# sqlp/sedumi

Hardware: AMD Instinct MI355X
Metric: IPM iters/sec (ADA' form+factor+solve) (higher is better)
Workload: dtype f64; 1 GPU; control07.mat: examples/control07.mat (BASELINE.json configs[1]), m=666, nnz(At)=107940, nnz(ADA')=443556, nnz(L)=222111; unit = getada1+2+3, blkchol, 4x(fwblkslv,./d,bwblkslv); parallelism=single GPU

## Files before the change

### sedumi_amd/csrc/sdm_ada.hip

```cpp
#include "sdm_plan.h"
#include <algorithm>
#include <cmath>
#include <cstdlib>

namespace sdm {

__global__ void k_dsqr(double *dsqr, const int *code, const double *dl, const double *ddet, int nlq) {
  int r = blockIdx.x * blockDim.x + threadIdx.x;
  if (r < nlq) { int c = code[r]; dsqr[r] = c == -1 ? dl[r] : (c >= 0 ? ddet[c] : -ddet[-2 - c]); }
}
__global__ void k_fill(double *x, double v, int64_t n) {
  int64_t t = (int64_t)blockIdx.x * blockDim.x + threadIdx.x;
  int64_t stride = (int64_t)gridDim.x * blockDim.x;
  for (; t < n; t += stride) x[t] = v;
}

constexpr int SPDOT_CAP = 2048;
template <int LPE>
__global__ void __launch_bounds__(256)
k_ada_spdot(double *ada, const int64_t *ADAjc, const int *ADAir, const int64_t *Mbeg, const int64_t *Mend,
            const int *Mir, const double *Mpr, const double *wgt, const int *invperm, int accumulate, int jbase, int cap) {
  SDM_DYN_SMEM(smem);
  double *jv = (double *)smem;
  int *jr = (int *)(jv + cap);
// ... 238 lines not shown
            if (part) { ar -= x * di; ai += x * dr; } else { ar += x * dr; ai += x * di; }
          }
        }
        Y[t * n + i] = ar;
        Dl[t * n + i] = D[(int64_t)col * n + i];
        if (herm) { Yi[t * n + i] = ai; Dli[t * n + i] = -Di[(int64_t)col * n + i]; }
      }
    }
    __syncthreads();
    if (!herm) {
      double sreg[S1_TREG];
#pragma unroll
      for (int k = 0; k < S1_TREG; k++) sreg[k] = 0.0;
#pragma unroll 1
      for (int t = 0; t < cc; t++) {
        const double *Yt = Y + t * n, *Dt = Dl + t * n;
#pragma unroll
        for (int k = 0; k < S1_TREG; k++) sreg[k] += Yt[rreg[k]] * Dt[creg[k]] + Yt[creg[k]] * Dt[rreg[k]];
      }
#pragma unroll
      for (int k = 0; k < S1_TREG; k++) zreg[k] += sreg[k] / 2;
    }
    for (int u = nreg + tid; u < ulen; u += bs) {
      int q = U[u];
      const int zpart = q >= n * n ? 1 : 0;
      q -= zpart * n * n;
      const int c = q / n, r = q - c * n;
      double v;
      if (!herm) {
        double a1 = 0.0, a2 = 0.0;
        for (int t = 0; t < cc; t++) {
          a1 += Y[t * n + r] * Dl[t * n + c];
          a2 += Y[t * n + c] * Dl[t * n + r];
        }
        v = (a1 + a2) / 2;
      } else {
        double rrc = 0.0, irc = 0.0, rcr = 0.0, icr = 0.0;
        for (int t = 0; t < cc; t++) {
          const double drc = Dl[t * n + c], dic = Dli[t * n + c], drr = Dl[t * n + r], dir = Dli[t * n + r];
          const double yr_r = Y[t * n + r], yi_r = Yi[t * n + r], yr_c = Y[t * n + c], yi_c = Yi[t * n + c];
          rrc += yr_r * drc - yi_r * dic; irc += yr_r * dic + yi_r * drc;
          rcr += yr_c * drr - yi_c * dir; icr += yr_c * dir + yi_c * drr;
        }
        v = zpart ? (irc - icr) / 2 : (rrc + rcr) / 2;
      }
      if (c0 == 0) z[u] = v; else z[u] += v;
    }
    __syncthreads();
  }
  if (!herm && R2.ada && ulen <= S1_TREG * bs) {
    double *zl = Y;
#pragma unroll
    for (int k = 0; k < S1_TREG; k++) if (tid + k * bs < ulen) zl[tid + k * bs] = zreg[k];
    __syncthreads();
    const int j = R2.t_col[task], kblk = T.t_blk[task];
    const int ipj = R2.invperm ? R2.invperm[j] : 0;
    for (int64_t e = R2.ADAjc[j] + tid; e < R2.ADAjc[j + 1]; e += bs) {
      const int i = R2.ADAir[e];
      if (R2.invperm && R2.invperm[i] > ipj) continue;
      double acc = 0.0, aabs = 0.0;
      int64_t p = R2.Ajc_psd[i];
      const int64_t pe = R2.Ajc[i + 1];
      for (; p + 4 <= pe; p += 4) {
        double x[4]; int b[4], u[4];
#pragma unroll
        for (int q = 0; q < 4; q++) { x[q] = R2.Apr[p + q]; b[q] = R2.Ablk[p + q]; u[q] = R2.Aupos[p + q]; }
#pragma unroll
        for (int q = 0; q < 4; q++) if (b[q] == kblk) { const double term = x[q] * zl[u[q]]; acc += term; aabs += fabs(term); }
      }
      for (; p < pe; p++) if (R2.Ablk[p] == kblk) { const double term = R2.Apr[p] * zl[R2.Aupos[p]]; acc += term; aabs += fabs(term); }
      const double base = R2.ada[e];
      R2.ada[e] = base + acc;
      if (i == j) R2.absd[j] = base + aabs;
    }
    return;
  }
  if (!herm) {
#pragma unroll
    for (int k = 0; k < S1_TREG; k++) if (tid + k * bs < ulen) z[tid + k * bs] = zreg[k];
  }
}

__global__ void __launch_bounds__(64 * S1_WAVES, 3 * S1_WAVES / 4)
k_psd_stage1_mfma(Stage1Tab T, const double *udsqr, double *zbuf, int ldsY, int nzcap, int task0, const int *order, double *zero_ptr, long long zero_n) {
  SDM_DYN_SMEM(smem);
  for (long long i = (long long)blockIdx.x * blockDim.x + threadIdx.x; i < zero_n; i += (long long)gridDim.x * blockDim.x) zero_ptr[i] = 0.0;
  const int task = order ? order[blockIdx.x] : blockIdx.x + task0;
  const int n = T.t_n[task], nslot = T.t_nslot[task], ulen = T.t_ulen[task];
  const int np = (n + 15) & ~15, nt = np >> 4, ntile = nt * nt;
  double *Yl = (double *)smem;
  double *Dl = Yl + S1_KC * np;
  double *Zl = (double *)smem;
  const int ldz = n | 1;
  const int64_t slot0 = T.t_slotptr[task], tend = T.t_end[task];
  const double *D = udsqr + T.t_udoff[task];
  double *z = zbuf + T.t_zoff[task];
  const int64_t rowbase = T.psd_start[T.t_blk[task]];
  const int tid = threadIdx.x, bs = blockDim.x;
  const int wave = SDM_UNIFORM_INT(tid >> 6), lane = tid & 63, nw = bs >> 6;
  const int li = lane & 15, lk = lane >> 4;
  const int rcpn = ((1 << 20) + n - 1) / n;
  static_assert(S1_KC * S1_MAXN * S1_MAXN < (1 << 20) && S1_KC % 4 == 0, "k_psd_stage1_mfma: reciprocal division, four slots per MFMA step");
  sdm_double4 acc[S1_MAXT];
  for (int x = 0; x < S1_MAXT; x++) for (int r = 0; r < 4; r++) acc[x][r] = 0.0;
  double *nzx = (double *)smem + ldsY;
  int *nzr = (int *)(nzx + nzcap);
  __shared__ int sbeg[S1_MAXN + 1], scol[S1_MAXN];
  SDM_PHASE_BEGIN();
  const int64_t nzb = T.s_nzptr[slot0];
  const bool staged = tend - nzb <= nzcap && nslot <= S1_MAXN;
  if (staged) {
    for (int64_t u = nzb + tid; u < tend; u += bs) { nzx[u - nzb] = T.Apr[u]; nzr[u - nzb] = (int)(T.Air[u] - rowbase); }
    for (int t = tid; t <= nslot; t += bs) sbeg[t] = (int)((t < nslot ? T.s_nzptr[slot0 + t] : tend) - nzb);
    for (int t = tid; t < nslot; t += bs) scol[t] = T.s_col[slot0 + t];
  }
  __syncthreads();
  SDM_PHASE(0);
  for (int t = wave; t < S1_KC; t += nw)
    if (lane < np - n) { Yl[t * np + n + lane] = 0.0; Dl[t * np + n + lane] = 0.0; }
  for (int c0 = 0; c0 < nslot; c0 += S1_KC) {
    const int cc = min(S1_KC, nslot - c0), kq = (cc + 3) & ~3;
    for (int e = tid; e < cc * n; e += bs) {
      const int t = (e * rcpn) >> 20, i = e - t * n;
      int sb, se, col;
      if (staged) { sb = sbeg[c0 + t]; se = sbeg[c0 + t + 1]; col = scol[c0 + t]; }
      else {
        sb = (int)(T.s_nzptr[slot0 + c0 + t] - nzb);
        se = (int)(((c0 + t + 1 < nslot) ? T.s_nzptr[slot0 + c0 + t + 1] : tend) - nzb);
        col = T.s_col[slot0 + c0 + t];
      }
      double a = 0.0;
      if (staged) {
        int u = sb;
        for (; u + 4 <= se; u += 4) {
          const double d0 = D[(int64_t)(nzr[u] - col * n) * n + i], d1 = D[(int64_t)(nzr[u + 1] - col * n) * n + i];
          const double d2 = D[(int64_t)(nzr[u + 2] - col * n) * n + i], d3 = D[(int64_t)(nzr[u + 3] - col * n) * n + i];
          a += nzx[u] * d0; a += nzx[u + 1] * d1; a += nzx[u + 2] * d2; a += nzx[u + 3] * d3;
        }
        for (; u < se; u++) a += nzx[u] * D[(int64_t)(nzr[u] - col * n) * n + i];
      } else {
        for (int64_t u = nzb + sb; u < nzb + se; u++) a += T.Apr[u] * D[(int64_t)((int)(T.Air[u] - rowbase) - col * n) * n + i];
      }
      Yl[t * np + i] = a;
      Dl[t * np + i] = D[(int64_t)col * n + i];
    }
    for (int t = cc + wave; t < kq; t += nw)
      for (int i = lane; i < n; i += 64) { Yl[t * np + i] = 0.0; Dl[t * np + i] = 0.0; }
    SDM_PHASE(1);
    __syncthreads();
    SDM_PHASE(2);
    for (int x = 0; x < S1_MAXT; x++) {
      const int tile = wave + x * nw;
      if (tile < ntile) {
        const int I = tile / nt, J = tile - I * nt;
        int npo = np; SDM_PIN(npo);
        const double *Ya = Yl + lk * npo + I * 16 + li, *Db = Dl + lk * npo + J * 16 + li;
        int q = 0;
        for (; q + 4 <= kq / 4; q += 4) {
          double a[4], b[4];
#pragma unroll
          for (int k = 0; k < 4; k++) { a[k] = Ya[4 * (q + k) * npo]; b[k] = Db[4 * (q + k) * npo]; }
#pragma unroll
          for (int k = 0; k < 4; k++) acc[x] = SDM_MFMA_F64_16x16x4(a[k], b[k], acc[x]);
        }
        for (; q < kq / 4; q++) acc[x] = SDM_MFMA_F64_16x16x4(Ya[4 * q * npo], Db[4 * q * npo], acc[x]);
      }
    }
    SDM_PHASE(3);
    __syncthreads();
    SDM_PHASE(4);
  }
  for (int x = 0; x < S1_MAXT; x++) {
    const int tile = wave + x * nw;
    if (tile < ntile) {
      const int I = tile / nt, J = tile - I * nt;
      for (int r = 0; r < 4; r++)
        if (I * 16 + lk + 4 * r < n && J * 16 + li < n) Zl[(I * 16 + lk + 4 * r) * ldz + J * 16 + li] = acc[x][r];
    }
  }
  __syncthreads();
  SDM_PHASE(5);
  const int *RC = T.u_rc + T.t_uoff[task];
  for (int u0 = 0; u0 < ulen; u0 += 8 * bs) {
    int rc[8];
#pragma unroll
    for (int x = 0; x < 8; x++) rc[x] = RC[min(u0 + x * bs + tid, ulen - 1)];
#pragma unroll
    for (int x = 0; x < 8; x++) {
      const int u = u0 + x * bs + tid;
      const int r = rc[x] >> 16, c = rc[x] & 0xffff;
      if (u < ulen) z[u] = (Zl[r * ldz + c] + Zl[c * ldz + r]) / 2;
    }
  }
  SDM_PHASE(6);
#if defined(SDM_PHASES) && !defined(SDM_EMU)
  if (tid == 0) { atomicAdd(&sdm_phase_acc[30], 1ull); if (n > 40) atomicAdd(&sdm_phase_acc[31], 1ull); }
#endif
}

__global__ void __launch_bounds__(256)
k_psd_stage2(double *ada, double *absd, const int64_t *ADAjc, const int *ADAir, const int64_t *Ajc,
             const int64_t *Ajc_psd, const double *Apr, const int *Ablk, const int *Aupos,
             const int64_t *c_taskptr, const int *t_blk, const int64_t *t_zoff, const int64_t *c_zlen, const double *zbuf,
             const int *invperm, int nblk, int thread_per_row, int jbase, int zlds) {
  SDM_DYN_SMEM(smem);
  long long *zo = (long long *)smem;
  double *zl = (double *)(zo + nblk);
  const int j = blockIdx.x + jbase;
  const int tid = threadIdx.x, bs = blockDim.x;
  const int64_t tb0 = c_taskptr[j], te0 = c_taskptr[j + 1];
  const bool jhas = te0 > tb0;
  const int64_t z0 = jhas ? t_zoff[tb0] : 0;
  const int64_t zlen = c_zlen[j];
  for (int k = tid; k < nblk; k += bs) zo[k] = -1;
  __syncthreads();
  for (int64_t t = tb0 + tid; t < te0; t += bs) zo[t_blk[t]] = t_zoff[t] - z0;
  const bool staged = thread_per_row && jhas && zlen <= zlds;
  if (staged)
    for (int64_t u = tid; u < zlen; u += bs) zl[u] = zbuf[z0 + u];
  __syncthreads();
  const double *zsrc = staged ? zl : zbuf + z0;
  const int ipj = invperm ? invperm[j] : 0;
  if (thread_per_row) {
    for (int64_t e = ADAjc[j] + tid; e < ADAjc[j + 1]; e += bs) {
      const int i = ADAir[e];
      if (invperm && invperm[i] > ipj) continue;
      double acc = 0.0, aabs = 0.0;
      if (jhas) {
        int64_t t = Ajc_psd[i];
        const int64_t te = Ajc[i + 1];
        for (; t + 4 <= te; t += 4) {
          double x[4]; int b[4], u[4];
#pragma unroll
          for (int q = 0; q < 4; q++) { x[q] = Apr[t + q]; b[q] = Ablk[t + q]; u[q] = Aupos[t + q]; }
#pragma unroll
          for (int q = 0; q < 4; q++) {
            const long long off = zo[b[q]];
            if (off >= 0) { const double term = x[q] * zsrc[off + u[q]]; acc += term; aabs += fabs(term); }
          }
        }
        for (; t < te; t++) {
          const long long off = zo[Ablk[t]];
          if (off >= 0) { const double term = Apr[t] * zsrc[off + Aupos[t]]; acc += term; aabs += fabs(term); }
        }
      }
      const double base = ada[e];
      ada[e] = base + acc;
      if (i == j) absd[j] = jhas ? base + aabs : 0.0;
    }
  } else {
    const int wave = tid >> 6, lane = tid & 63, nw = bs >> 6;
    for (int64_t e = ADAjc[j] + wave; e < ADAjc[j + 1]; e += nw) {
      const int i = ADAir[e];
      if (invperm && invperm[i] > ipj) continue;
      double acc = 0.0, aabs = 0.0;
      if (jhas)
        for (int64_t t = Ajc_psd[i] + lane; t < Ajc[i + 1]; t += 64) {
          const long long off = zo[Ablk[t]];
          if (off >= 0) { const double term = Apr[t] * zsrc[off + Aupos[t]]; acc += term; aabs += fabs(term); }
        }
      for (int off = 32; off > 0; off >>= 1) { acc += __shfl_down(acc, off); aabs += __shfl_down(aabs, off); }
      if (lane == 0) {
        const double base = ada[e];
        ada[e] = base + acc;
        if (i == j) absd[j] = jhas ? base + aabs : 0.0;
// ... 423 lines not shown
}
static Stage1Tab stage1_tab(const AdaPlan &A) {
  Stage1Tab T;
  T.t_n = A.t_n.p; T.t_nslot = A.t_nslot.p; T.t_ulen = A.t_ulen.p; T.t_herm = A.t_herm.p; T.s_col = A.s_col.p;
  T.u_pos = A.u_pos.p; T.u_rc = A.u_rc.p; T.Air = A.d_Air.p; T.t_slotptr = A.t_slotptr.p; T.t_udoff = A.t_udoff.p; T.t_uoff = A.t_uoff.p;
  T.t_zoff = A.t_zoff.p; T.t_end = A.t_end.p; T.s_nzptr = A.s_nzptr.p; T.Apr = A.d_Apr.p; T.t_blk = A.t_blk.p;
  T.psd_start = A.d_psd_start.p;
  return T;
}
static Stage2Ride stage2_ride(sdm_plan *P, double *ada, const int *d_invperm) {
  const AdaPlan &A = P->ada;
  Stage2Ride R2 = {};
  R2.ada = ada; R2.absd = P->absd.p; R2.ADAjc = A.d_ADAjc.p; R2.Ajc = A.d_Ajc.p; R2.Ajc_psd = A.d_Ajc_psd.p; R2.ADAir = A.d_ADAir.p;
  R2.Ablk = A.d_Ablk.p; R2.Aupos = A.d_Aupos.p; R2.t_col = A.t_col.p; R2.invperm = d_invperm; R2.Apr = A.d_Apr.p;
  return R2;
}
template <int JB>
static void launch_stage2_ell(sdm_plan *P, double *ada, const int *d_invperm, int ncols, int jbase, bool sym, int gsplit, bool cleared) {
  AdaPlan &A = P->ada;
  const size_t lds = (size_t)JB * (size_t)A.zmax * sizeof(double);
#ifndef SDM_EMU
  if (lds > 48 * 1024) SDM_HIP_CHECK(hipFuncSetAttribute((const void *)k_psd_stage2_ell<JB>, hipFuncAttributeMaxDynamicSharedMemorySize, (int)lds));
#endif
  SDM_KLAUNCH_AS(P, P->stream, JB == 4 ? "k_psd_stage2_ell<4>" : JB == 2 ? "k_psd_stage2_ell<2>" : "k_psd_stage2_ell<1>", k_psd_stage2_ell<JB>,
                 dim3((ncols + JB - 1) / JB, gsplit), dim3(64 * ELL_WAVES), lds, ada, P->absd.p, A.d_ADAjc.p, A.d_ADAir.p,
                 A.d_Ajc.p, A.d_Ajc_psd.p, A.d_Apr.p, A.d_Ablk.p, A.d_Aupos.p, A.c_taskptr.p, A.t_blk.p, A.t_ulen.p,
                 A.t_zoff.p, A.zbuf.p, A.d_uoff.p, A.g_row.p, A.g_len.p, A.g_off.p, A.g_val.p, A.g_bu.p, A.ell_ng, d_invperm,
                 (int)A.zmax, (int)A.m, jbase, jbase + ncols, A.ell_pos.p, sym ? (const int *)A.ell_order.p : (const int *)nullptr,
                 A.d_Azpos.p, A.t_zdst.p, cleared ? 1 : 0,
                 sym ? (const long long *)A.cdp64.p : (const long long *)A.cdc64.p, sym ? (const int *)A.cdp32.p : (const int *)A.cdc32.p);
}
void ada_psd(sdm_plan *P, double *ada, const int *d_invperm, bool sym_input, bool absd_done) {
  AdaPlan &A = P->ada;
  const int m = (int)A.m;
  if (A.sdpN == 0 || sym_input || A.col1 <= A.col0) ada_zero_flush(P);
  if (A.sdpN == 0) {
    if (sym_input) symmetrize_in_place(P, ada);
    if (!absd_done) SDM_KLAUNCH(P, k_diag, dim3((m + 255) / 256), dim3(256), 0, P->absd.p, ada, A.d_ADAjc.p, A.d_ADAir.p, m);
    return;
  }
  if (A.col1 <= A.col0) return;
  const int ncols = (int)(A.col1 - A.col0), jbase = (int)A.col0;
  const int task0 = (int)A.h_taskptr[A.col0], ntask = (int)(A.h_taskptr[A.col1] - A.h_taskptr[A.col0]);
  const size_t direct_lds = (size_t)(2 * A.sdpN + 2 * S1_DIRECT_MAXNZ * A.sdpN + 2) * sizeof(int) + (size_t)(2 * A.sdpN) * sizeof(long long) +
                            (size_t)(S1_DIRECT_MAXNZ * A.sdpN) * sizeof(double);
  const bool direct = A.thread_per_row && !A.ell_ok && A.sdpN == A.rsdpN && A.s1_maxnz <= S1_DIRECT_MAXNZ && direct_lds <= S1_DIRECT_LDS_MAX;
  const bool direct_zero = direct && !sym_input && !d_invperm && A.zero_ptr == ada + P->ada_jc[A.col0] &&
                           A.zero_n == (long long)(P->ada_jc[A.col1] - P->ada_jc[A.col0]);
  if (direct_zero) { A.zero_ptr = nullptr; A.zero_n = 0; }
  const bool s1_mfma = A.maxn <= S1_MAXN && A.sdpN == A.rsdpN;
  if (direct || ntask <= 0 || !s1_mfma) ada_zero_flush(P);
  if (direct) {
    if (sym_input) symmetrize_in_place(P, ada);
    const int nb = (int)A.sdpN;
    const size_t lds_cols = (size_t)DIRECT_JB * (direct_lds + 16) + (size_t)A.sdpN * sizeof(int);
    if (!d_invperm && (int64_t)(P->ada_jc[A.col1] - P->ada_jc[A.col0]) == (int64_t)ncols * m && lds_cols <= S1_DIRECT_LDS_MAX) {
      const int ysplit = std::max(1, std::min(16, (int)((m + 511) / 512)));
      SDM_KLAUNCH(P, k_psd_direct_cols, dim3((ncols + DIRECT_JB - 1) / DIRECT_JB, ysplit), dim3(256), lds_cols, ada, P->absd.p, A.d_ADAjc.p, A.d_Ajc.p, A.d_Ajc_psd.p, A.d_Apr.p,
                  A.d_Air.p, A.d_Ablk.p, A.c_taskptr.p, A.t_blk.p, A.t_n.p, A.t_udoff.p, A.t_slotptr.p, A.s_nzptr.p, A.t_end.p, A.d_psd_start.p, A.udsqr.p,
                  nb, jbase, jbase + ncols, m, direct_zero ? 1 : 0);
    } else
      SDM_KLAUNCH(P, k_psd_direct, dim3(ncols), dim3(256), direct_lds, ada, P->absd.p, A.d_ADAjc.p, A.d_ADAir.p, A.d_Ajc.p, A.d_Ajc_psd.p, A.d_Apr.p, A.d_Air.p,
                  A.d_Ablk.p, A.c_taskptr.p, A.t_blk.p, A.t_n.p, A.t_udoff.p, A.t_slotptr.p, A.s_nzptr.p, A.t_end.p, A.d_psd_start.p, A.udsqr.p,
                  d_invperm, nb, jbase, direct_zero ? 1 : 0);
    SDM_HIP_CHECK(hipGetLastError());
    return;
  }
  bool stage1_cleared_all = false;
  if (ntask > 0) {
    const Stage1Tab T = stage1_tab(A);
#ifndef SDM_EMU
    SDM_HIP_CHECK(hipFuncSetAttribute((const void *)k_psd_stage1, hipFuncAttributeMaxDynamicSharedMemorySize, (int)A.stage1_lds));
#endif
    const int nzcap = s1_nzcap(A.s1_maxnz);
    if (s1_mfma) {
      const int ldsy = s1_mfma_ldsy(A.maxn);
      const size_t lds = s1_mfma_lds(A.maxn, A.s1_maxnz);
#ifndef SDM_EMU
      if (lds > 48 * 1024) SDM_HIP_CHECK(hipFuncSetAttribute((const void *)k_psd_stage1_mfma, hipFuncAttributeMaxDynamicSharedMemorySize, (int)lds));
#endif
      double *zp = A.zero_ptr; const long long zn = A.zero_n;
      A.zero_ptr = nullptr; A.zero_n = 0;
      stage1_cleared_all = zp == ada + P->ada_jc[A.col0] && zn == (long long)(P->ada_jc[A.col1] - P->ada_jc[A.col0]);
      SDM_KLAUNCH(P, k_psd_stage1_mfma, dim3((unsigned)ntask), dim3(64 * S1_WAVES), lds, T, A.udsqr.p, A.zbuf.p, ldsy, nzcap, task0,
                  (ntask == (int)A.ntask) ? (const int *)A.t_order.p : (const int *)nullptr, zp, zn);
    } else {
      const size_t one = (size_t)(A.sdpN > A.rsdpN ? 4 : 2) * (size_t)A.maxn * sizeof(double);
      const size_t ldsy = std::max(one, std::min(A.stage1_lds, (size_t)S1_GEN_LDS));
      const size_t lds = ldsy + (size_t)nzcap * (sizeof(double) + sizeof(int));
#ifndef SDM_EMU
      SDM_HIP_CHECK(hipFuncSetAttribute((const void *)k_psd_stage1, hipFuncAttributeMaxDynamicSharedMemorySize, (int)lds));
#endif
      const bool ride = A.one_task_per_col && A.thread_per_row && !A.ell_ok && A.sdpN == A.rsdpN && A.s1_maxulen <= 6 * 512 &&
                        (int64_t)A.s1_maxulen * (int64_t)sizeof(double) <= (int64_t)ldsy;
      if (ride) {
        if (sym_input) symmetrize_in_place(P, ada);
        SDM_HIP_CHECK(hipMemsetAsync(P->absd.p + jbase, 0, (size_t)ncols * sizeof(double), P->stream));
      }
      SDM_KLAUNCH(P, k_psd_stage1, dim3((unsigned)ntask), dim3(512), lds, T, A.udsqr.p, A.zbuf.p, (int)(ldsy / sizeof(double)), task0, nzcap,
                  ride ? stage2_ride(P, ada, d_invperm) : Stage2Ride{},
                  (ntask == (int)A.ntask && A.t_order_xcd.n == (size_t)ntask) ? (const int *)A.t_order_xcd.p : (const int *)nullptr);
      if (ride) { SDM_HIP_CHECK(hipGetLastError()); return; }
    }
  }
  if (sym_input) symmetrize_in_place(P, ada);
  if (A.ell_ok) {
    const bool sym = A.ell_full && !d_invperm && jbase == 0 && ncols == m;
    const int gsplit = sym ? 3 : 1;
    const bool cleared = stage1_cleared_all && !sym_input;
    const size_t zbytes = (size_t)A.zmax * sizeof(double);
    if (4 * zbytes <= 64 * 1024 && m >= 1024) launch_stage2_ell<4>(P, ada, d_invperm, ncols, jbase, sym, gsplit, cleared);
    else if (2 * zbytes <= 64 * 1024 && m >= 512) launch_stage2_ell<2>(P, ada, d_invperm, ncols, jbase, sym, gsplit, cleared);
    else launch_stage2_ell<1>(P, ada, d_invperm, ncols, jbase, sym, gsplit, cleared);
  } else {
    const int64_t zl = (A.thread_per_row && A.zmaxj * 8 <= 64 * 1024) ? A.zmaxj : 0;
    const size_t lds = (size_t)A.sdpN * 8 + (size_t)zl * 8;
#ifndef SDM_EMU
    if (lds > 48 * 1024) SDM_HIP_CHECK(hipFuncSetAttribute((const void *)k_psd_stage2, hipFuncAttributeMaxDynamicSharedMemorySize, (int)lds));
#endif
    SDM_KLAUNCH(P, k_psd_stage2, dim3(ncols), dim3(256), lds, ada, P->absd.p, A.d_ADAjc.p, A.d_ADAir.p, A.d_Ajc.p,
               A.d_Ajc_psd.p, A.d_Apr.p, A.d_Ablk.p, A.d_Aupos.p, A.c_taskptr.p, A.t_blk.p, A.t_zoff.p, A.c_zlen.p, A.zbuf.p,
               d_invperm, (int)A.sdpN, A.thread_per_row ? 1 : 0, jbase, (int)zl);
  }
  SDM_HIP_CHECK(hipGetLastError());
}

}

#if defined(SDM_PHASES) && !defined(SDM_EMU)
extern "C" int sdm_debug_phases_ada(unsigned long long *out32, int reset) {
  if (out32 && hipMemcpyFromSymbol(out32, HIP_SYMBOL(sdm_phase_acc), 32 * sizeof(unsigned long long)) != hipSuccess) return 1;
  if (reset) { unsigned long long z[32] = {0}; if (hipMemcpyToSymbol(HIP_SYMBOL(sdm_phase_acc), z, sizeof(z)) != hipSuccess) return 1; }
  return 0;
}
#endif
```

### sedumi_amd/csrc/sdm_ada_build.hip

```cpp
#include "sdm_plan.h"
#include <algorithm>

namespace sdm {
namespace {

struct AdaIn {
  sdm_int m; const sdm_int *Ajc, *Air; const double *Apr; const sdm_int *Ajc_psd;
  sdm_int lpN, lorN, sdpN, rsdpN; const sdm_int *sdpNL, *qblkstart, *psd_blkstart, *Qjc, *Qir, *ADAjc, *ADAir;
  sdm_int psd_begin(sdm_int j) const { return sdpN > 0 ? Ajc_psd[j] : Ajc[j + 1]; }
};
struct PsdPatterns {
  std::vector<int> Ablk, Aupos;
  std::vector<std::vector<int>> U;
  std::vector<int64_t> uoff;
  sdm_int psdnnz = 0;
};
struct Stage1Tasks {
  std::vector<int> t_col, t_blk, t_n, t_nslot, t_ulen, t_herm, s_col, order, order_xcd;
  std::vector<int64_t> t_slotptr, t_udoff, t_uoff, t_zoff, t_end, s_nzptr, c_taskptr, c_zlen;
};

void upload_narrow(DevBuf<int> &d, const sdm_int *h, sdm_int n) { std::vector<int> v((size_t)n); for (sdm_int t = 0; t < n; t++) v[t] = (int)h[t]; d.upload(v); }

PsdPatterns psd_patterns(AdaPlan &A, const AdaIn &in) {
// ... 152 lines not shown
    }
  A.ell_ng = ng;
  A.g_row.upload(grow); A.g_len.upload(glen); A.g_off.upload(goff); A.g_val.upload(gval); A.g_bu.upload(gbu);
  { std::vector<int> pos((size_t)m); for (sdm_int p = 0; p < m; p++) pos[(size_t)order[p]] = (int)p; A.ell_pos.upload(pos); }
  A.ell_order.upload(order);
  A.ell_full = (in.ADAjc[m] == (sdm_int)m * m);
  A.d_uoff.upload(pt.uoff); A.d_Azpos.upload(zp); A.t_zdst.upload(zd);
  ell_column_records(in, tk, zd, nullptr, A.cdc64, A.cdc32);
  ell_column_records(in, tk, zd, order.data(), A.cdp64, A.cdp32);
  A.ell_ok = true;
}

std::vector<int> ada_transpose_map(const AdaIn &in) {
  const sdm_int m = in.m, *ADAjc = in.ADAjc, *ADAir = in.ADAir;
  std::vector<int> adaT((size_t)ADAjc[m], -1);
  for (sdm_int j = 0; j < m; j++)
    for (sdm_int e = ADAjc[j]; e < ADAjc[j + 1]; e++) {
      sdm_int i = ADAir[e];
      const sdm_int *b = ADAir + ADAjc[i], *en = ADAir + ADAjc[i + 1];
      const sdm_int *f = std::lower_bound(b, en, j);
      if (f != en && *f == j) adaT[e] = (int)(f - ADAir);
    }
  return adaT;
}

void lq_dense_forms(AdaPlan &A, const AdaIn &in) {
  const sdm_int m = in.m, lorN = in.lorN;
  sdm_int nz = 0;
  for (sdm_int j = 0; j < m; j++) nz += in.Ajc_psd[j] - in.Ajc[j];
  const double cells = (double)A.nlq * (double)m;
  A.lq_dense = A.nlq > 0 && m > 1 && nz > 0 && (double)nz >= 0.10 * cells && cells * 8.0 <= 1.0e9;
  A.q_dense = lorN > 0 && A.nnzQ > 0 && (double)A.nnzQ >= 0.10 * (double)lorN * (double)m && (double)lorN * m * 8.0 <= 1.0e9;
  if (A.lq_dense) {
    std::vector<double> D((size_t)A.nlq * (size_t)m, 0.0);
    for (sdm_int j = 0; j < m; j++)
      for (sdm_int t = in.Ajc[j]; t < in.Ajc_psd[j]; t++) D[(size_t)j * (size_t)A.nlq + (size_t)in.Air[t]] = in.Apr[t];
    A.Alq_d.upload(D);
  } else A.Alq_d.release();
  if (A.q_dense) {
    std::vector<int64_t> dst((size_t)A.nnzQ);
    for (sdm_int j = 0; j < m; j++)
      for (sdm_int t = in.Qjc[j]; t < in.Qjc[j + 1]; t++) dst[(size_t)t] = (int64_t)j * lorN + in.Qir[t];
    A.q_dst.upload(dst);
    A.Q_d.alloc((size_t)lorN * (size_t)m);
    if (A.lq_dense && (double)lorN * (double)m <= 1.6e7) {
      std::vector<int> src((size_t)lorN * (size_t)m, -1);
      for (sdm_int t = 0; t < A.nnzQ; t++) src[(size_t)dst[(size_t)t]] = (int)t;
      A.q_src.upload(src);
    } else A.q_src.release();
  } else { A.Q_d.release(); A.q_dst.release(); A.q_src.release(); }
  if (A.lq_dense || A.q_dense) {
    const int nt = (int)((m + TILE - 1) / TILE), T = nt * (nt + 1) / 2;
    const sdm_int rows = std::max(A.lq_dense ? A.nlq : 0, A.q_dense ? lorN : 0);
    A.gram_split = (int)std::max<sdm_int>(1, std::min<sdm_int>((rows + TILE - 1) / TILE, std::max(1, 512 / T)));
    A.gram_part.alloc((size_t)A.gram_split * (size_t)m * (size_t)m);
  } else A.gram_part.release();
}

void upload_tables(AdaPlan &A, const AdaIn &in, const PsdPatterns &pt, const Stage1Tasks &tk, const std::vector<int> &adaT) {
  const sdm_int m = in.m, lorN = in.lorN, sdpN = in.sdpN;
  { std::vector<int> code((size_t)A.nlq, -1);
    for (sdm_int r = in.lpN; r < in.lpN + lorN && r < A.nlq; r++) code[r] = (int)(-2 - (r - in.lpN));
    for (sdm_int k = 0; k < lorN; k++)
      for (sdm_int r = in.qblkstart[k]; r < in.qblkstart[k + 1] && r < A.nlq; r++) code[r] = (int)k;
    A.dsqr_code.upload(code); }
  A.d_Ajc.upload(in.Ajc, (size_t)m + 1); A.d_Ajc_psd.upload(in.Ajc_psd, (size_t)m);
  upload_narrow(A.d_Air, in.Air, A.nnzA);
  A.d_Apr.upload(in.Apr, (size_t)A.nnzA);
  A.d_Ablk.upload(pt.Ablk); A.d_Aupos.upload(pt.Aupos);
  { std::vector<int64_t> v(m + 1, 0); if (lorN > 0) v.assign(in.Qjc, in.Qjc + m + 1); A.d_Qjc.upload(v); }
  upload_narrow(A.d_Qir, in.Qir, A.nnzQ);
  A.d_ADAjc.upload(in.ADAjc, (size_t)m + 1);
  upload_narrow(A.d_ADAir, in.ADAir, in.ADAjc[m]);
  A.d_ADAT.upload(adaT);
  { std::vector<int> upos((size_t)pt.uoff[sdpN]), urc(upos.size(), 0);
    for (sdm_int k = 0; k < sdpN; k++) std::copy(pt.U[k].begin(), pt.U[k].end(), upos.begin() + pt.uoff[k]);
    for (sdm_int k = 0; k < std::min(sdpN, in.rsdpN); k++) {
      const int n = (int)A.psd_n[k];
      if (n >= 65536) continue;
      for (size_t u = 0; u < pt.U[k].size(); u++) { const int q = pt.U[k][u], c = q / n, r = q - c * n; urc[(size_t)pt.uoff[k] + u] = (r << 16) | c; }
    }
    A.u_pos.upload(upos); A.u_rc.upload(urc); }
  A.t_col.upload(tk.t_col); A.t_blk.upload(tk.t_blk); A.t_n.upload(tk.t_n); A.t_nslot.upload(tk.t_nslot); A.t_ulen.upload(tk.t_ulen);
  A.t_herm.upload(tk.t_herm); A.t_order.upload(tk.order);
  if (tk.order_xcd.empty()) A.t_order_xcd.release(); else A.t_order_xcd.upload(tk.order_xcd);
  A.t_slotptr.upload(tk.t_slotptr); A.t_udoff.upload(tk.t_udoff); A.t_uoff.upload(tk.t_uoff); A.t_zoff.upload(tk.t_zoff);
  A.s_col.upload(tk.s_col); A.s_nzptr.upload(tk.s_nzptr); A.c_taskptr.upload(tk.c_taskptr); A.c_zlen.upload(tk.c_zlen);
  A.t_end.upload(tk.t_end);
  { std::vector<int64_t> v(A.psd_start.begin(), A.psd_start.end()); if (v.empty()) v.push_back(0); A.d_psd_start.upload(v); }
  { std::vector<int64_t> v(lorN + 1, A.nlq); for (sdm_int k = 0; k <= lorN && lorN > 0; k++) v[k] = in.qblkstart[k]; A.d_qblk.upload(v); }
  A.zbuf.alloc((size_t)std::max<int64_t>(A.zlen, 1));
  A.dsqr.alloc((size_t)std::max<sdm_int>(A.nlq, 1));
  A.dl.alloc((size_t)std::max<sdm_int>(in.lpN, 1)); A.ddet.alloc((size_t)std::max<sdm_int>(lorN, 1));
  A.qpr.alloc((size_t)std::max<sdm_int>(A.nnzQ, 1)); A.udsqr.alloc((size_t)std::max<sdm_int>(A.lenud, 1));
  A.q1.alloc((size_t)std::max<sdm_int>(lorN, 1));
  A.q2.alloc((size_t)std::max<sdm_int>(lorN > 0 ? in.qblkstart[lorN] - in.qblkstart[0] : 0, 1));
  A.symtmp.alloc((size_t)std::max<sdm_int>(in.ADAjc[m], 1));
  const size_t need = (size_t)(sdpN > in.rsdpN ? 4 : 2) * (size_t)A.maxn * sizeof(double);
  A.stage1_lds = std::max<size_t>(96 * 1024, need);
  if (A.stage1_lds > 136 * 1024) throw std::runtime_error("PSD block too large for the LDS-staged D*A*D kernel (n > 8700)");
}

}

void ada_build(sdm_plan *P, sdm_int N, sdm_int m, const sdm_int *Ajc, const sdm_int *Air, const double *Apr, const sdm_int *Ajc_psd, sdm_int lpN,
               sdm_int lorN, sdm_int sdpN, sdm_int rsdpN, const sdm_int *sdpNL, const sdm_int *qblkstart, const sdm_int *psd_blkstart,
               const sdm_int *Qjc, const sdm_int *Qir, const sdm_int *ADAjc, const sdm_int *ADAir) {
  AdaPlan &A = P->ada;
  const AdaIn in = {m, Ajc, Air, Apr, Ajc_psd, lpN, lorN, sdpN, rsdpN, sdpNL, qblkstart, psd_blkstart, Qjc, Qir, ADAjc, ADAir};
  A.N = N; A.m = m; A.nnzA = Ajc[m]; A.lpN = lpN; A.lorN = lorN; A.sdpN = sdpN; A.rsdpN = rsdpN;
  A.ic_n.release(); A.ufac.release();
  if (A.nnzA >= (sdm_int)1 << 31 || N >= (sdm_int)1 << 31) throw std::runtime_error("At too large for 32-bit row indices");
  A.nlq = sdpN > 0 ? psd_blkstart[0] : N;
  if (lorN > 0 && qblkstart[lorN] != A.nlq && sdpN > 0) throw std::runtime_error("qblkstart / psd_blkstart mismatch");
  const PsdPatterns pt = psd_patterns(A, in);
  A.thread_per_row = (m > 0 && pt.psdnnz / (double)m < 48.0);
  A.nnz_lq = A.nnzA - pt.psdnnz;
  A.nnzQ = lorN > 0 ? Qjc[m] : 0;
  A.lq_maxcol = 0; A.q_maxcol = 0;
  for (sdm_int j = 0; j < m; j++) A.lq_maxcol = std::max<int64_t>(A.lq_maxcol, in.psd_begin(j) - Ajc[j]);
  for (sdm_int j = 0; j < m && lorN > 0; j++) A.q_maxcol = std::max<int64_t>(A.q_maxcol, Qjc[j + 1] - Qjc[j]);
  const Stage1Tasks tk = stage1_tasks(A, in, pt);
  stage2_ell(A, in, pt, tk);
  upload_tables(A, in, pt, tk, ada_transpose_map(in));
  lq_dense_forms(A, in);
  P->has_ada = true;
}

}
```

### sedumi_amd/csrc/sdm_plan.h

```cpp
#pragma once
#include "../../include/sedumi_hip.h"
#include "sdm_rt.h"
#include <mutex>
#include <string>
#include <vector>

namespace sdm {

constexpr int NB = 64;
constexpr int TILE = 64;
constexpr int UTP = 72;
constexpr int S1_MAXN = 96;
constexpr int S1_KC = 32;
constexpr int S1_WAVES = 8;
constexpr int S1_NZ = 1536;
constexpr int s1_nzcap(int64_t maxnz) { return (int)(((maxnz + 1) & ~(int64_t)1) < S1_NZ ? ((maxnz + 1) & ~(int64_t)1) : S1_NZ); }
constexpr int s1_mfma_ldsy(int maxn) { return 2 * S1_KC * ((maxn + 15) & ~15) > maxn * (maxn | 1) ? 2 * S1_KC * ((maxn + 15) & ~15) : maxn * (maxn | 1); }
constexpr size_t s1_mfma_lds(int maxn, int64_t maxnz) { return (size_t)s1_mfma_ldsy(maxn) * sizeof(double) + (size_t)s1_nzcap(maxnz) * (sizeof(double) + sizeof(int)); }
constexpr int S1_MAXT = ((S1_MAXN / 16) * (S1_MAXN / 16) + S1_WAVES - 1) / S1_WAVES;
constexpr int S1_GEN_LDS = 74 * 1024;
constexpr int ELL_WAVES = 8;
constexpr int SOLVE_LDS_MAX = 3072;
constexpr int FUSE_MAX_TILES = 1 << 20;
constexpr int SBW_MIN = 256;
constexpr int SBW_MAX = 2048;
constexpr int SINV_MAXLEV = 4;
constexpr int SPREP_NCNT = 2 + 2 * SINV_MAXLEV;
constexpr int SROWS = 16;
#ifndef SDM_SW
#define SDM_SW 8
#endif
constexpr int SW = SDM_SW;
constexpr int LDL_THREADS = 512;
constexpr int PANEL_THREADS = 256;
constexpr int ROWS_BATCH = 16 * (PANEL_THREADS / 64);
constexpr int TRSM_ROWS = 128;
#ifndef SDM_MFMA_MIN_ROWS
#define SDM_MFMA_MIN_ROWS 48
#endif
constexpr int MFMA_MIN_ROWS = SDM_MFMA_MIN_ROWS;
constexpr int CHK = 16;
constexpr int64_t ASM_FULL_MAX = 4 << 20;
constexpr int FRONT_MAXT = 64;
constexpr int FRONT_XCNT_OFF = 2 * FRONT_MAXT + FRONT_MAXT * FRONT_MAXT;
constexpr int FRONT_CNT = FRONT_XCNT_OFF + FRONT_MAXT * FRONT_MAXT;
constexpr int FRONT_POOL = 1;
constexpr int PANEL_RB = (LDL_THREADS / 64) * NB * 17;
constexpr size_t PANEL_LDS = (size_t)(NB * (NB + 1) + PANEL_RB) * sizeof(double);
constexpr size_t PANEL_LDS_RIDE = std::max(PANEL_LDS, (size_t)4 * NB * UTP * sizeof(double));
constexpr int FRONT_CV_OFF = NB * (NB + 1) + (LDL_THREADS / 64) * NB * 17;
constexpr size_t FRONT_LDS = (size_t)(FRONT_CV_OFF + NB * TILE) * sizeof(double);
static_assert(PANEL_RB >= NB * NB && PANEL_RB >= (NB - CHK) * TRSM_ROWS && TRSM_ROWS == 16 * (LDL_THREADS / 64) && ROWS_BATCH <= TRSM_ROWS, "panel LDS layout");

template <class T>
struct DevBuf {
  T *p = nullptr;
  size_t n = 0;
  DevBuf() = default;
  DevBuf(const DevBuf &) = delete;
  DevBuf &operator=(const DevBuf &) = delete;
  DevBuf(DevBuf &&o) noexcept : p(o.p), n(o.n) { o.p = nullptr; o.n = 0; }
  DevBuf &operator=(DevBuf &&o) noexcept { if (this != &o) { release(); p = o.p; n = o.n; o.p = nullptr; o.n = 0; } return *this; }
  ~DevBuf() { release(); }
  void release() {
    if (p) (void)hipFree(p);
    p = nullptr; n = 0;
  }
  void alloc(size_t count) {
    release();
    n = count;
    SDM_HIP_CHECK(hipMalloc((void **)&p, (count ? count : 1) * sizeof(T)));
  }
  void upload(const std::vector<T> &h) {
    alloc(h.size());
    if (!h.empty()) SDM_HIP_CHECK(hipMemcpy(p, h.data(), h.size() * sizeof(T), hipMemcpyHostToDevice));
  }
  void upload(const T *h, size_t count) {
    alloc(count);
    if (count) SDM_HIP_CHECK(hipMemcpy(p, h, count * sizeof(T), hipMemcpyHostToDevice));
  }
};

struct PanelCtx {
  double *lb; const double *ubp; int *pivstat; double *pivval; double *colbuf; const double *ada; const int *asm_src; const int64_t *Ljc;
  int mtot, pad;
};

struct HostFlag {
  int *host = nullptr;
  HostFlag() = default;
  HostFlag(const HostFlag &) = delete;
  HostFlag &operator=(const HostFlag &) = delete;
  HostFlag(HostFlag &&o) noexcept : host(o.host) { o.host = nullptr; }
  HostFlag &operator=(HostFlag &&o) noexcept { if (this != &o) { if (host) (void)hipHostFree(host); host = o.host; o.host = nullptr; } return *this; }
  ~HostFlag() { if (host) (void)hipHostFree(host); }
  void ensure() {
    if (host) return;
    SDM_HIP_CHECK(hipHostMalloc((void **)&host, 4 * sizeof(int), 0));
    for (int i = 0; i < 4; i++) host[i] = 0;
  }
  int *dev() {
    ensure();
// ... 46 lines not shown
  std::vector<int> childptr, childlist, levptr, levlist, lev_T;
  std::vector<char> sn_active;
  double pars_canceltol = 0, pars_maxu = 0, pars_abstol = 0; int pars_use_absd = 0;
  bool begun = false;
  std::vector<LevelLaunch> launches;
  std::vector<int> lev_first_launch;
  DevBuf<int> d_first, d_ns, d_ms, d_ld, d_parent, d_childptr, d_childlist, d_levlist, d_lindx, d_relidx, d_perm;
  DevBuf<int64_t> d_foff, d_xl, d_woff, d_roff, d_toff, d_asm_dst, d_asm_dstT, d_Ljc;
  DevBuf<int> d_asm_src;
  DevBuf<double> fronts, frontsT, wvec, colbuf, d, dsolve, lb, pivval, ub;
  DevBuf<int> pivstat;
  DevBuf<int> diag_cnt;
  DevBuf<int> d_asm_fsrc;
  DevBuf<int> front_cnt;
  DevBuf<int> d_fslot;
  std::vector<char> lev_persist;
  std::vector<int> lev_maxT;
  std::vector<int> lev_ntw;
  DevBuf<int> upd_cnt;
  DevBuf<double> panelrec;
  DevBuf<PanelCtx> panel_ctx;
  PanelCtx panel_ctx_host = {};
  HostFlag tmo;
  int *sweep_tmo() { return tmo.dev() + 1; }
  int sbw = SBW_MIN;
  int sbw_req = 0;
  bool front_off_req = false;
  bool sprep_off = false;
  int tile_wgs_req = 0;
  int64_t ssize = 0; int nsbtot = 0;
  std::vector<int64_t> sn_soff; std::vector<int> sn_sld, sn_sboff;
  DevBuf<int64_t> d_soff; DevBuf<int> d_sld, d_sboff;
  DevBuf<double> S, xfin, zdiv;
  DevBuf<double> ST;
  DevBuf<double> LT;
  std::vector<int64_t> sn_ltoff; DevBuf<int64_t> d_ltoff;
  DevBuf<int> l_lt; int n_lt = 0;
  DevBuf<double> Tarena;
  DevBuf<int> sweep_cnt;
  DevBuf<unsigned long long> sb_g;
  DevBuf<int> l_i128, l_items;
  int n_i128 = 0, n_items = 0;
  bool follow = false;
  bool front_disabled = false;
  bool merge_disabled = false;
  std::vector<int> lev_followT;
  std::vector<int> stage_ptr;
  std::vector<SolveLevel> slev;
  DevBuf<double> prep_part; DevBuf<int> prep_ticket;
  double growth_max = 1e4;
  double growth_used = 1e4;
  double refine_max = 1e10;
  int refine_mode = 1;
  bool refine_on = false;
  int sweep_seq = 0;
  HostFlag noted;
};

struct FrontTab {
  const int *first, *ns, *ms, *ld;
  const int64_t *foff, *xl, *woff, *roff, *toff;
  const int *childptr, *childlist, *lindx, *relidx;
  const int64_t *soff; const int *sld, *sboff;
  const int64_t *ltoff = nullptr;
  const int *fslot = nullptr;
  int one = 0, o_s = 0, o_ns = 0, o_ms = 0, o_ld = 0, o_first = 0, o_sld = 0, o_sboff = 0;
  int64_t o_foff = 0, o_soff = 0, o_woff = 0, o_xl = 0, o_ltoff = 0;
};

struct AdaPlan {
  sdm_int N = 0, m = 0, nnzA = 0, lpN = 0, lorN = 0, sdpN = 0, rsdpN = 0;
  sdm_int nlq = 0;
  sdm_int lenud = 0, ntask = 0, zlen = 0, nnzQ = 0, nnz_lq = 0;
  int maxn = 0;
  bool thread_per_row = false;
  sdm_int col0 = 0, col1 = 0;
  double *zero_ptr = nullptr; long long zero_n = 0; bool zero_defer = false;
  std::vector<int64_t> h_taskptr;
  std::vector<sdm_int> psd_n, psd_start, psd_udoff;
  DevBuf<int64_t> d_Ajc, d_Ajc_psd, d_Qjc, d_ADAjc;
  DevBuf<int> d_Air, d_Qir, d_ADAir, d_ADAT;
  DevBuf<double> d_Apr;
  DevBuf<int> d_Ablk, d_Aupos;
  DevBuf<int> t_col, t_blk, t_n, t_nslot, t_ulen, t_herm, t_order, t_order_xcd;
  DevBuf<int64_t> t_slotptr, t_udoff, t_uoff, t_zoff;
  DevBuf<int> s_col;
  DevBuf<int64_t> s_nzptr;
  int64_t s1_maxnz = 0;
  int64_t lq_maxcol = 0, q_maxcol = 0;
  bool one_task_per_col = false;
  int s1_maxulen = 0;
  DevBuf<int> u_rc;
  DevBuf<int> u_pos;
  DevBuf<int64_t> c_taskptr;
  DevBuf<double> zbuf, dsqr, symtmp;
  DevBuf<int> dsqr_code;
  bool lq_dense = false, q_dense = false;
  int gram_split = 1;
  DevBuf<double> Alq_d, Q_d, gram_part;
  DevBuf<int64_t> q_dst;
  DevBuf<int> q_src;
  DevBuf<int64_t> t_end, d_psd_start;
  DevBuf<double> dl, ddet, qpr, udsqr;
  DevBuf<double> q1, q2;
  DevBuf<int64_t> d_qblk;
  DevBuf<double> ufac;
  DevBuf<int> ic_n, ic_poff, ic_perm; DevBuf<int64_t> ic_off;
  PinnedInts ic_perm_host; bool ic_has_perm = false;
  std::vector<sdm_int> h_Ajc, h_Air; std::vector<double> h_Apr;
  bool pcg_ready = false;
  DevBuf<int64_t> d_Tjc, pb_off; DevBuf<int> d_Tir, pb_n, pb_herm, pb_poff, pb_items, aden_cols;
  DevBuf<double> d_Tpr, xN, psd, psdtmp, aden;
  int pcg_ntiles = 0, aden_n = 0;
  DevBuf<double> wp_rv, wp_rb, qauxdet, qauxtr, wp_y, wp_dx, wp_r, wp_work, wp_part, wp_sc;
  PinnedInts wp_host;
  size_t stage1_lds = 0;
  bool ell_ok = false;
  int ell_ng = 0;
  int64_t zmax = 0, zmaxj = 0;
  DevBuf<int64_t> c_zlen;
  DevBuf<int> g_row, g_len, g_bu;
  DevBuf<long long> cdc64, cdp64;
  DevBuf<int> cdc32, cdp32;
  DevBuf<int> d_Azpos, t_zdst;
  DevBuf<int> ell_pos;
  DevBuf<int> ell_order;
  bool ell_full = false;
  DevBuf<int64_t> g_off, d_uoff;
  DevBuf<double> g_val;
};

}

namespace sdm {
struct KProf {
  bool enabled = false;
  struct Rec { const char *name; hipEvent_t a, b; };
  std::vector<Rec> recs;
  std::vector<hipEvent_t> pool;
  hipEvent_t get() {
    if (!pool.empty()) { hipEvent_t e = pool.back(); pool.pop_back(); return e; }
    hipEvent_t e; SDM_HIP_CHECK(hipEventCreate(&e)); return e;
  }
};
}

namespace sdm {
struct DensePlan {
  sdm_int nden = 0, dznnz = 0, pnnz = 0, mrows = 0;
  bool active = false, factored = false;
  bool tables_on_host = false;
  std::vector<sdm_int> LADjc, LADir, dzjc, dzir, colperm, first;
  std::vector<int64_t> poff, betajc, permoff;
  std::vector<int> dopiv;
  std::vector<int> later_ptr;
  DevBuf<int> d_dzir, d_colperm, d_pivperm, d_dopiv, d_later;
  DevBuf<int64_t> d_dzjc, d_poff, d_betajc, d_permoff;
  DevBuf<double> ad, lad, wvb, p, beta, dgat, smult, dden;
  DevBuf<double> w_psq, w_mu, w_key;
  DevBuf<int> w_ord, w_ord2, w_acc, w_post, w_dep, w_st;
};
}

struct sdm_plan {
  int device = 0;
  sdm::DensePlan dense;
  sdm::KProf kprof;
// ... 171 lines not shown
```

Before: 2828 IPM iters/s.

## Pack stage-1 task metadata into 64-byte records and prefetch D gathers

Per-task metadata for the PSD stage-1 MFMA kernel now lives in one 64-byte record, with an array pre-permuted into the launch order. Each block does a single contiguous load instead of a chain of dependent gathers through order, t_* and psd_start. The staged gather loop is software-pipelined so the next element's first D value and diagonal are fetched while the current one accumulates. It also moves index arithmetic to 32-bit unsigned offsets, which assumes the offsets fit in 32 bits.

```diff
diff --git a/sedumi_amd/csrc/sdm_ada.hip b/sedumi_amd/csrc/sdm_ada.hip
--- a/sedumi_amd/csrc/sdm_ada.hip
+++ b/sedumi_amd/csrc/sdm_ada.hip
@@ -344,23 +344,21 @@
 }
 
 __global__ void __launch_bounds__(64 * S1_WAVES, 3 * S1_WAVES / 4)
-k_psd_stage1_mfma(Stage1Tab T, const double *udsqr, double *zbuf, int ldsY, int nzcap, int task0, const int *order, double *zero_ptr, long long zero_n) {
+k_psd_stage1_mfma(Stage1Tab T, const S1Rec *recs, const double *udsqr, double *zbuf, int ldsY, int nzcap, int rec0, double *zero_ptr, long long zero_n) {
   SDM_DYN_SMEM(smem);
   for (long long i = (long long)blockIdx.x * blockDim.x + threadIdx.x; i < zero_n; i += (long long)gridDim.x * blockDim.x) zero_ptr[i] = 0.0;
-  const int task = order ? order[blockIdx.x] : blockIdx.x + task0;
-  const int n = T.t_n[task], nslot = T.t_nslot[task], ulen = T.t_ulen[task];
+  const S1Rec rec = recs[blockIdx.x + rec0];
+  const int n = rec.n, nslot = rec.nslot, ulen = rec.ulen;
   const int np = (n + 15) & ~15, nt = np >> 4, ntile = nt * nt;
   double *Yl = (double *)smem;
   double *Dl = Yl + S1_KC * np;
   double *Zl = (double *)smem;
   const int ldz = n | 1;
-  const int64_t slot0 = T.t_slotptr[task], tend = T.t_end[task];
-  const double *D = udsqr + T.t_udoff[task];
-  double *z = zbuf + T.t_zoff[task];
-  const int64_t rowbase = T.psd_start[T.t_blk[task]];
+  const int slot0 = rec.slot0, tend = rec.tend, rowbase = rec.rowbase;
+  const double *D = udsqr + rec.udoff;
+  double *z = zbuf + rec.zoff;
   const int tid = threadIdx.x, bs = blockDim.x;
   const int wave = SDM_UNIFORM_INT(tid >> 6), lane = tid & 63, nw = bs >> 6;
-  const int li = lane & 15, lk = lane >> 4;
   const int rcpn = ((1 << 20) + n - 1) / n;
   static_assert(S1_KC * S1_MAXN * S1_MAXN < (1 << 20) && S1_KC % 4 == 0, "k_psd_stage1_mfma: reciprocal division, four slots per MFMA step");
   sdm_double4 acc[S1_MAXT];
@@ -369,10 +367,10 @@
   int *nzr = (int *)(nzx + nzcap);
   __shared__ int sbeg[S1_MAXN + 1], scol[S1_MAXN];
   SDM_PHASE_BEGIN();
-  const int64_t nzb = T.s_nzptr[slot0];
+  const int nzb = rec.nzb;
   const bool staged = tend - nzb <= nzcap && nslot <= S1_MAXN;
   if (staged) {
-    for (int64_t u = nzb + tid; u < tend; u += bs) { nzx[u - nzb] = T.Apr[u]; nzr[u - nzb] = (int)(T.Air[u] - rowbase); }
+    for (int u = nzb + tid; u < tend; u += bs) { nzx[u - nzb] = T.Apr[u]; nzr[u - nzb] = T.Air[u] - rowbase; }
     for (int t = tid; t <= nslot; t += bs) sbeg[t] = (int)((t < nslot ? T.s_nzptr[slot0 + t] : tend) - nzb);
     for (int t = tid; t < nslot; t += bs) scol[t] = T.s_col[slot0 + t];
   }
@@ -382,32 +380,55 @@
     if (lane < np - n) { Yl[t * np + n + lane] = 0.0; Dl[t * np + n + lane] = 0.0; }
   for (int c0 = 0; c0 < nslot; c0 += S1_KC) {
     const int cc = min(S1_KC, nslot - c0), kq = (cc + 3) & ~3;
-    for (int e = tid; e < cc * n; e += bs) {
-      const int t = (e * rcpn) >> 20, i = e - t * n;
-      int sb, se, col;
-      if (staged) { sb = sbeg[c0 + t]; se = sbeg[c0 + t + 1]; col = scol[c0 + t]; }
-      else {
-        sb = (int)(T.s_nzptr[slot0 + c0 + t] - nzb);
-        se = (int)(((c0 + t + 1 < nslot) ? T.s_nzptr[slot0 + c0 + t + 1] : tend) - nzb);
-        col = T.s_col[slot0 + c0 + t];
-      }
-      double a = 0.0;
-      if (staged) {
+    const int ne = cc * n;
+    if (staged) {
+#define S1_D(x) (*(const double *)((const char *)D + (unsigned)((x) * 8)))
+      auto fetch = [&](int e_, int &yo_, int &off_, int &sb_, int &se_, double &p_, double &dl_) {
+        const int t_ = (e_ * rcpn) >> 20, i_ = e_ - t_ * n;
+        const int cn_ = scol[c0 + t_] * n;
+        sb_ = sbeg[c0 + t_]; se_ = sbeg[c0 + t_ + 1];
+        yo_ = t_ * np + i_; off_ = i_ - cn_ * n;
+        p_ = S1_D(nzr[sb_] * n + off_);
+        dl_ = S1_D(cn_ + i_);
+      };
+      int e = tid, yo = 0, off = 0, sb = 0, se = 0;
+      SDM_PIN(e);
+      double p = 0.0, dl = 0.0;
+      if (e < ne) fetch(e, yo, off, sb, se, p, dl);
+      while (e < ne) {
+        const int e2 = e + bs;
+        int yo2 = 0, off2 = 0, sb2 = 0, se2 = 0;
+        double p2 = 0.0, dl2 = 0.0;
+        if (e2 < ne) fetch(e2, yo2, off2, sb2, se2, p2, dl2);
+        double a = 0.0;
         int u = sb;
-        for (; u + 4 <= se; u += 4) {
-          const double d0 = D[(int64_t)(nzr[u] - col * n) * n + i], d1 = D[(int64_t)(nzr[u + 1] - col * n) * n + i];
-          const double d2 = D[(int64_t)(nzr[u + 2] - col * n) * n + i], d3 = D[(int64_t)(nzr[u + 3] - col * n) * n + i];
+        a += nzx[u] * p;
+        for (u++; u + 4 <= se; u += 4) {
+          const double d0 = S1_D(nzr[u] * n + off), d1 = S1_D(nzr[u + 1] * n + off), d2 = S1_D(nzr[u + 2] * n + off), d3 = S1_D(nzr[u + 3] * n + off);
           a += nzx[u] * d0; a += nzx[u + 1] * d1; a += nzx[u + 2] * d2; a += nzx[u + 3] * d3;
         }
-        for (; u < se; u++) a += nzx[u] * D[(int64_t)(nzr[u] - col * n) * n + i];
-      } else {
-        for (int64_t u = nzb + sb; u < nzb + se; u++) a += T.Apr[u] * D[(int64_t)((int)(T.Air[u] - rowbase) - col * n) * n + i];
-      }
-      Yl[t * np + i] = a;
-      Dl[t * np + i] = D[(int64_t)col * n + i];
-    }
+        for (; u < se; u++) a += nzx[u] * S1_D(nzr[u] * n + off);
+        Yl[yo] = a;
+        Dl[yo] = dl;
+        e = e2; yo = yo2; off = off2; sb = sb2; se = se2; p = p2; dl = dl2;
+      }
+#undef S1_D
+    } else {
+      for (int e = tid; e < ne; e += bs) {
+        const int t = (e * rcpn) >> 20, i = e - t * n;
+        const int sb = (int)(T.s_nzptr[slot0 + c0 + t] - nzb);
+        const int se = (int)(((c0 + t + 1 < nslot) ? T.s_nzptr[slot0 + c0 + t + 1] : (int64_t)tend) - nzb);
+        const int col = T.s_col[slot0 + c0 + t];
+        double a = 0.0;
+        for (int u = nzb + sb; u < nzb + se; u++) a += T.Apr[u] * D[(int64_t)((T.Air[u] - rowbase) - col * n) * n + i];
+        Yl[t * np + i] = a;
+        Dl[t * np + i] = D[(int64_t)col * n + i];
+      }
+    }
+    int lane_c = lane; SDM_PIN(lane_c);
+    const int li = lane_c & 15, lk = lane_c >> 4;
     for (int t = cc + wave; t < kq; t += nw)
-      for (int i = lane; i < n; i += 64) { Yl[t * np + i] = 0.0; Dl[t * np + i] = 0.0; }
+      for (int i = lane_c; i < n; i += 64) { Yl[t * np + i] = 0.0; Dl[t * np + i] = 0.0; }
     SDM_PHASE(1);
     __syncthreads();
     SDM_PHASE(2);
@@ -432,6 +453,8 @@
     __syncthreads();
     SDM_PHASE(4);
   }
+  int lane_z = lane; SDM_PIN(lane_z);
+  const int li = lane_z & 15, lk = lane_z >> 4;
   for (int x = 0; x < S1_MAXT; x++) {
     const int tile = wave + x * nw;
     if (tile < ntile) {
@@ -442,7 +465,7 @@
   }
   __syncthreads();
   SDM_PHASE(5);
-  const int *RC = T.u_rc + T.t_uoff[task];
+  const int *RC = T.u_rc + rec.uoff;
   for (int u0 = 0; u0 < ulen; u0 += 8 * bs) {
     int rc[8];
 #pragma unroll
@@ -1032,8 +1055,9 @@
       double *zp = A.zero_ptr; const long long zn = A.zero_n;
       A.zero_ptr = nullptr; A.zero_n = 0;
       stage1_cleared_all = zp == ada + P->ada_jc[A.col0] && zn == (long long)(P->ada_jc[A.col1] - P->ada_jc[A.col0]);
-      SDM_KLAUNCH(P, k_psd_stage1_mfma, dim3((unsigned)ntask), dim3(64 * S1_WAVES), lds, T, A.udsqr.p, A.zbuf.p, ldsy, nzcap, task0,
-                  (ntask == (int)A.ntask) ? (const int *)A.t_order.p : (const int *)nullptr, zp, zn);
+      const bool all = ntask == (int)A.ntask;
+      SDM_KLAUNCH(P, k_psd_stage1_mfma, dim3((unsigned)ntask), dim3(64 * S1_WAVES), lds, T, all ? (const S1Rec *)A.s1_rec_order.p : (const S1Rec *)A.s1_rec.p,
+                  A.udsqr.p, A.zbuf.p, ldsy, nzcap, all ? 0 : task0, zp, zn);
     } else {
       const size_t one = (size_t)(A.sdpN > A.rsdpN ? 4 : 2) * (size_t)A.maxn * sizeof(double);
       const size_t ldsy = std::max(one, std::min(A.stage1_lds, (size_t)S1_GEN_LDS));
diff --git a/sedumi_amd/csrc/sdm_ada_build.hip b/sedumi_amd/csrc/sdm_ada_build.hip
--- a/sedumi_amd/csrc/sdm_ada_build.hip
+++ b/sedumi_amd/csrc/sdm_ada_build.hip
@@ -258,11 +258,21 @@
     }
     A.u_pos.upload(upos); A.u_rc.upload(urc); }
   A.t_col.upload(tk.t_col); A.t_blk.upload(tk.t_blk); A.t_n.upload(tk.t_n); A.t_nslot.upload(tk.t_nslot); A.t_ulen.upload(tk.t_ulen);
-  A.t_herm.upload(tk.t_herm); A.t_order.upload(tk.order);
+  A.t_herm.upload(tk.t_herm);
   if (tk.order_xcd.empty()) A.t_order_xcd.release(); else A.t_order_xcd.upload(tk.order_xcd);
   A.t_slotptr.upload(tk.t_slotptr); A.t_udoff.upload(tk.t_udoff); A.t_uoff.upload(tk.t_uoff); A.t_zoff.upload(tk.t_zoff);
   A.s_col.upload(tk.s_col); A.s_nzptr.upload(tk.s_nzptr); A.c_taskptr.upload(tk.c_taskptr); A.c_zlen.upload(tk.c_zlen);
   A.t_end.upload(tk.t_end);
+  { std::vector<S1Rec> rec((size_t)A.ntask), rec_order((size_t)A.ntask);
+    for (sdm_int t = 0; t < A.ntask; t++) {
+      S1Rec &r = rec[(size_t)t];
+      r = S1Rec{};
+      r.n = tk.t_n[t]; r.nslot = tk.t_nslot[t]; r.ulen = tk.t_ulen[t]; r.slot0 = (int)tk.t_slotptr[t]; r.tend = (int)tk.t_end[t];
+      r.nzb = (int)tk.s_nzptr[(size_t)tk.t_slotptr[t]]; r.rowbase = (int)A.psd_start[(size_t)tk.t_blk[t]];
+      r.udoff = tk.t_udoff[t]; r.zoff = tk.t_zoff[t]; r.uoff = tk.t_uoff[t];
+    }
+    for (sdm_int x = 0; x < A.ntask; x++) rec_order[(size_t)x] = rec[(size_t)tk.order[(size_t)x]];
+    A.s1_rec.upload(rec); A.s1_rec_order.upload(rec_order); }
   { std::vector<int64_t> v(A.psd_start.begin(), A.psd_start.end()); if (v.empty()) v.push_back(0); A.d_psd_start.upload(v); }
   { std::vector<int64_t> v(lorN + 1, A.nlq); for (sdm_int k = 0; k <= lorN && lorN > 0; k++) v[k] = in.qblkstart[k]; A.d_qblk.upload(v); }
   A.zbuf.alloc((size_t)std::max<int64_t>(A.zlen, 1));
diff --git a/sedumi_amd/csrc/sdm_plan.h b/sedumi_amd/csrc/sdm_plan.h
--- a/sedumi_amd/csrc/sdm_plan.h
+++ b/sedumi_amd/csrc/sdm_plan.h
@@ -18,6 +18,11 @@
 constexpr int s1_mfma_ldsy(int maxn) { return 2 * S1_KC * ((maxn + 15) & ~15) > maxn * (maxn | 1) ? 2 * S1_KC * ((maxn + 15) & ~15) : maxn * (maxn | 1); }
 constexpr size_t s1_mfma_lds(int maxn, int64_t maxnz) { return (size_t)s1_mfma_ldsy(maxn) * sizeof(double) + (size_t)s1_nzcap(maxnz) * (sizeof(double) + sizeof(int)); }
 constexpr int S1_MAXT = ((S1_MAXN / 16) * (S1_MAXN / 16) + S1_WAVES - 1) / S1_WAVES;
+struct S1Rec {
+  int n, nslot, ulen, slot0, tend, nzb, rowbase, pad0;
+  long long udoff, zoff, uoff, pad1;
+};
+static_assert(sizeof(S1Rec) == 64, "S1Rec: one 64-byte record per task");
 constexpr int S1_GEN_LDS = 74 * 1024;
 constexpr int ELL_WAVES = 8;
 constexpr int SOLVE_LDS_MAX = 3072;
@@ -230,7 +235,8 @@
   DevBuf<int> d_Air, d_Qir, d_ADAir, d_ADAT;
   DevBuf<double> d_Apr;
   DevBuf<int> d_Ablk, d_Aupos;
-  DevBuf<int> t_col, t_blk, t_n, t_nslot, t_ulen, t_herm, t_order, t_order_xcd;
+  DevBuf<int> t_col, t_blk, t_n, t_nslot, t_ulen, t_herm, t_order_xcd;
+  DevBuf<S1Rec> s1_rec, s1_rec_order;
   DevBuf<int64_t> t_slotptr, t_udoff, t_uoff, t_zoff;
   DevBuf<int> s_col;
   DevBuf<int64_t> s_nzptr;
```

Result: no change. 2824 IPM iters/s (-0.1%).
